# kan-bayashi/espnet

Measured on AMD Instinct MI355X. Metric: frames/sec, 12L Conformer hybrid CTC/attention training step (B=32 T=1000 d=256 per GPU), higher is better.
Workload: dtype f32; 1 GPU; BASELINE configs[1]: 12L Conformer enc d=256 h=4 ff=2048 k=31 macaron+cnn rel_pos, 6L Transformer dec, V=5000, fbank B=32 T=1000 L=100, mtlalpha 0.3, lsm 0.1; global_batch=32, frames=1000, parallelism=dp1, optimizer=adam+noam, clip 5.0, launch=hipGraph, wgrad_side_stream=False, optimizer_steps_done=114

## Files before the change

### espnet_amd/_lib.py

```python
import ctypes as C
import os

import torch

_HERE = os.path.dirname(os.path.abspath(__file__))
LIB_PATH = os.path.join(_HERE, "csrc", "libespnet_amd_hip.so")


class EamdError(RuntimeError):
    pass


class GatherT(C.Structure):
    _fields_ = [("enabled", C.c_int32), ("C", C.c_int32), ("ntap", C.c_int32), ("Ho", C.c_int32),
                ("Wo", C.c_int32), ("Hin", C.c_int32), ("Win", C.c_int32), ("sh", C.c_int32),
                ("sw", C.c_int32), ("dh", C.c_int32 * 9), ("dw", C.c_int32 * 9)]


class RowMapT(C.Structure):
    _fields_ = [("enabled", C.c_int32), ("Ho", C.c_int32), ("Wo", C.c_int32), ("Hc", C.c_int32),
                ("Wc", C.c_int32), ("sh", C.c_int32), ("oh", C.c_int32), ("sw", C.c_int32),
                ("ow", C.c_int32)]


# ... 49 lines not shown
                ("lnb_x", C.c_void_p), ("lnb_gamma", C.c_void_p), ("lnb_mean", C.c_void_p), ("lnb_rstd", C.c_void_p),
                ("lnb_dres", C.c_void_p), ("lnb_ws", C.c_void_p), ("lnb_drop_out", C.c_void_p), ("lnb_drop_salt", C.c_uint64)]


class FfnPackT(C.Structure):
    _fields_ = [("w1", C.c_void_p), ("w2", C.c_void_p), ("fwd_first", C.c_void_p), ("fwd_second", C.c_void_p),
                ("bwd_first", C.c_void_p), ("bwd_second", C.c_void_p), ("D", C.c_int32), ("F", C.c_int32)]


class RowProjPackT(C.Structure):
    _fields_ = [("w", C.c_void_p), ("image", C.c_void_p), ("K", C.c_int32), ("N", C.c_int32), ("ldw", C.c_int32),
                ("trans", C.c_int32)]


class LstmSeqFwdT(C.Structure):
    _fields_ = [("gx", C.c_void_p), ("w_hh", C.c_void_p), ("b_hh", C.c_void_p), ("live", C.c_void_p),
                ("h_out", C.c_void_p), ("c_out", C.c_void_p), ("y", C.c_void_p), ("acts", C.c_void_p),
                ("reverse", C.c_int32), ("reserved", C.c_int32)]


class LstmSeqBwdT(C.Structure):
    _fields_ = [("dy", C.c_void_p), ("w_t", C.c_void_p), ("acts", C.c_void_p), ("c_out", C.c_void_p),
                ("live", C.c_void_p), ("dgates", C.c_void_p), ("reverse", C.c_int32), ("reserved", C.c_int32)]


_lib = None

SYMBOLS = [
    "eamd_abi_version", "eamd_gemm", "eamd_gemm_multi", "eamd_gemm_group_plan", "eamd_gemm_group_launch", "eamd_ffn_fwd", "eamd_ffn_bwd", "eamd_ffn_pack_f32", "eamd_ffn_pack_bf16", "eamd_ffn_pack_f32_multi", "eamd_rowproj", "eamd_rowproj_pack_f32", "eamd_rowproj_lnb_workspace", "eamd_layernorm_fwd", "eamd_layernorm_bwd_workspace", "eamd_layernorm_bwd_drop_f32", "eamd_layernorm_bwd", "eamd_layernorm_bwd_reduce", "eamd_attn_fwd", "eamd_attn_bwd_q", "eamd_attn_fwd_f32", "eamd_attn_bwd_q_f32", "eamd_attn_bwd_kv_f32", "eamd_attn_bwd_kv", "eamd_softmax_fwd",
    "eamd_softmax_bwd", "eamd_lsm_loss", "eamd_argmax_rows", "eamd_reduce_sum", "eamd_log_softmax_rows", "eamd_transducer_expand_rows", "eamd_topk_rows", "eamd_topk_rows_i32", "eamd_weighted_topk_rows", "eamd_beam_step", "eamd_beam_step_dyn", "eamd_decode_self_attn_dyn", "eamd_beam_slots_dyn", "eamd_ctc_prefix_psi_dyn", "eamd_ctc_prefix_state_dyn", "eamd_embed_pe_dyn", "eamd_copy_jobs", "eamd_embed_pe_ld", "eamd_linear_rows_f32", "eamd_linear_rows_ln_f32", "eamd_decode_self_attn", "eamd_beam_slots", "eamd_decode_src_attn", "eamd_decode_src_attn_group", "eamd_decode_src_attn_split", "eamd_decode_src_attn_split_workspace", "eamd_weighted_sum", "eamd_beam_select", "eamd_beam_finish",
    "eamd_axpby", "eamd_cast_bf16", "eamd_scale_dev", "eamd_act_fwd", "eamd_act_bwd", "eamd_glu_fwd", "eamd_glu_bwd",
    "eamd_add_bias2", "eamd_add_cast_bf16", "eamd_add_block_f32", "eamd_add_cast_colsum2", "eamd_add_colsum2_f32", "eamd_colsum", "eamd_embed_pe", "eamd_embed_bwd", "eamd_posenc", "eamd_posenc_scaled", "eamd_posenc_scaled_bwd", "eamd_permute4",
    "eamd_dropout", "eamd_rng_advance", "eamd_dwconv_fwd", "eamd_dwconv_glu_fwd", "eamd_dwconv_glu_bwd_x", "eamd_dwconv_glu_bwd_w", "eamd_dwconv_bwd_x", "eamd_dwconv_bwd_w", "eamd_bn_nslab",
    "eamd_bn_stats", "eamd_bn_finalize", "eamd_bn_apply", "eamd_bn_bwd", "eamd_bn_stats_bounded", "eamd_bn_bwd_bounded", "eamd_mask_time", "eamd_conv1_fwd", "eamd_conv1_bwd_w_workspace", "eamd_conv1_bwd_w",
    "eamd_conv2_weight_prep", "eamd_conv2_weight_grad", "eamd_add_sos_eos", "eamd_ctc_collapse",
    "eamd_ctc_workspace_bytes", "eamd_ctc_loss", "eamd_ctc_pit_workspace_bytes", "eamd_ctc_pit_loss", "eamd_ctc_align_workspace_bytes", "eamd_ctc_forced_align", "eamd_maskctc_seed", "eamd_maskctc_update", "eamd_ctc_prefix_score", "eamd_ctc_prefix_score_batch", "eamd_ctc_prefix_psi", "eamd_ctc_prefix_state", "eamd_grad_norm", "eamd_sched_step", "eamd_adam_step", "eamd_adadelta_step", "eamd_add_gradient_noise",
    "eamd_specaug", "eamd_global_mvn", "eamd_utterance_mvn", "eamd_reflect_pad", "eamd_logmel", "eamd_unfold1d", "eamd_fold1d", "eamd_attloc_convmax_fwd", "eamd_attloc_convmax_bwd", "eamd_layernorm_bwd_drop",
    "eamd_lstm_cell_fwd", "eamd_lstm_cell_bwd", "eamd_lstm_step_fwd", "eamd_lstm_step_bwd", "eamd_lstm_seq_sync_bytes", "eamd_lstm_seq_fwd", "eamd_lstm_seq_bwd", "eamd_lstm_seq_status", "eamd_lstm_seq_status_merge", "eamd_gru_cell_fwd", "eamd_gru_cell_bwd", "eamd_maxpool2x2_fwd", "eamd_maxpool2x2_bwd", "eamd_mask_rows",
    "eamd_joint_fwd", "eamd_joint_bwd", "eamd_rnnt_workspace", "eamd_rnnt_loss", "eamd_rnnt_grad", "eamd_rnnt_node_stats", "eamd_rnnt_node_stats_part", "eamd_rnnt_row_coef", "eamd_rnnt_alpha_beta", "eamd_rnnt_node_grad",
    "eamd_conv3x3_c1_fwd", "eamd_conv3x3_c1_bwd_w_workspace", "eamd_conv3x3_c1_bwd_w", "eamd_attloc_fwd", "eamd_attloc_bwd_energy", "eamd_attloc_bwd_workspace", "eamd_attloc_bwd_energy_conv", "eamd_attloc_bwd_conv",
    "eamd_att_dot_energy_fwd", "eamd_att_dot_energy_bwd", "eamd_att_ctx_fwd", "eamd_att_ctx_bwd",
]


def lib():
    global _lib
    if _lib is None:
        if not os.path.exists(LIB_PATH):
            raise EamdError(
                f"{LIB_PATH} not found: build it with `python -c 'import __graft_entry__ as g; g.build()'` "
                "or `make -C espnet_amd/csrc` (there is no CPU fallback)")
        _lib = C.CDLL(LIB_PATH)
        _lib.eamd_ctc_workspace_bytes.restype = C.c_int64
        _lib.eamd_ctc_align_workspace_bytes.restype = C.c_int64
        _lib.eamd_ctc_pit_workspace_bytes.restype = C.c_int64
        _lib.eamd_layernorm_bwd_workspace.restype = C.c_int64
        _lib.eamd_rnnt_workspace.restype = C.c_int64
        _lib.eamd_attloc_bwd_workspace.restype = C.c_int64
        _lib.eamd_conv1_bwd_w_workspace.restype = C.c_int64
        _lib.eamd_lstm_seq_sync_bytes.restype = C.c_int64
        _lib.eamd_conv3x3_c1_bwd_w_workspace.restype = C.c_int64
        for s in SYMBOLS:
            getattr(_lib, s)
    return _lib


_raw_stream = getattr(torch._C, "_cuda_getCurrentRawStream", None)
_cur_device = getattr(torch._C, "_cuda_getDevice", None)


def stream_ptr():
    if _raw_stream is not None and _cur_device is not None:
        return C.c_void_p(_raw_stream(_cur_device()))
    return C.c_void_p(torch.cuda.current_stream().cuda_stream)


EAMD_EUNSUPPORTED = -2


def check(rc, what):
    if rc != 0:
        raise EamdError(f"{what} failed with code {rc}")


def ptr(t, offset=0):
    if t is None:
        return None
    if not t.is_cuda:
        raise EamdError("espnet_amd kernels need GPU tensors (no CPU fallback in the product path)")
    if offset == 0:
        return C.c_void_p(t.data_ptr())
    return C.c_void_p(t.data_ptr() + offset * t.element_size())


# ... 5 lines not shown
```

### espnet_amd/csrc/convmod.hip

```cpp
#include <stdlib.h>
#include "common.h"
#include "../../include/espnet_amd.h"

namespace {

constexpr int KMAX = 32;

__device__ __forceinline__ void chan_merge(float& n, float& mean, float& m2, float nb, float mb, float m2b);

template <int NWV, int MODE>
__global__ __launch_bounds__(NWV * 64) void dwconv_lds_kernel(const float* __restrict__ x, const float* __restrict__ w,
                                                              const float* __restrict__ bias, float* __restrict__ y,
                                                              int B, int T, int C, int K, int pad, int flip,
                                                              const float* __restrict__ aglu, int y_bf16,
                                                              float* __restrict__ bn_part) {
  constexpr int TB = NWV * 8;
  constexpr int NR = (TB + KMAX - 1 + NWV - 1) / NWV;
  constexpr int NWL = (64 * KMAX + NWV * 64 - 1) / (NWV * 64);
  __shared__ float xs[(TB + KMAX - 1) * 64];
  __shared__ float wl[64 * KMAX];
  const int lane = threadIdx.x & 63, wave = threadIdx.x >> 6;
  const int c0 = blockIdx.x * 64;
  const int c = min(c0 + lane, C - 1);
  const int nblk = (T + TB - 1) / TB;
// ... 402 lines not shown
  }
  sh[0][t] = s1; sh[1][t] = s2;
  __syncthreads();
  if (gi == 0 && c < C) {
    for (int g2 = 1; g2 < BN_G; ++g2) { s1 += sh[0][g2 * BN_CPB + cl]; s2 += sh[1][g2 * BN_CPB + cl]; }
    sums[c] = s1; sums[C + c] = s2;
    dbeta[c] += s1; dgamma[c] += s2;
  }
}
__global__ void bn_bwd_apply_kernel(const float* __restrict__ dy, const float* __restrict__ x,
                                    const float* __restrict__ mean, const float* __restrict__ rstd,
                                    const float* __restrict__ gamma, const float* __restrict__ beta,
                                    const float* __restrict__ sums, float* __restrict__ dx, long M, int C, int act,
                                    int training, int T, const int* __restrict__ bound) {
  const long n = M * C;
  const long stride = (long)gridDim.x * blockDim.x;
  const int tb = bound ? bound[0] : T;
  const float invM = bound ? 1.f / ((float)(M / T) * (float)tb) : 1.f / (float)M;
  for (long i = (long)blockIdx.x * blockDim.x + threadIdx.x; i < n; i += stride) {
    int c = i % C;
    if (bound && (int)((i / C) % T) >= tb) { dx[i] = 0.f; continue; }
    float rs = rstd[c], g = gamma[c];
    float xh = (x[i] - mean[c]) * rs;
    float z = xh * g + beta[c];
    float d = dy[i];
    if (act == EAMD_ACT_SWISH) d *= eamd_dswish(z);
    else if (act == EAMD_ACT_RELU) d = z > 0.f ? d : 0.f;
    else if (act != EAMD_ACT_NONE) d *= eamd_dact(z, act);
    if (training) dx[i] = g * rs * (d - sums[c] * invM - xh * sums[C + c] * invM);
    else dx[i] = g * rs * d;
  }
}

constexpr int C1_MAXF = 512;
template <int ST, int NC>
__global__ __launch_bounds__(256) void conv1_fwd_kernel(const float* __restrict__ x, const float* __restrict__ w,
                                                        const float* __restrict__ bias, float* __restrict__ y, int B,
                                                        int T, int F, int H, int W, int C, int bf16, int pad) {
  constexpr int XLD = C1_MAXF + 32;
  constexpr int NV = (ST * 7 + 3 + 3) / 4;
  __shared__ __attribute__((aligned(16))) float xs[3 * XLD];
  const int row = blockIdx.x;
  const int b = row / H, hh = row % H;
  const int FP = F + 2 * pad;
  for (int i = threadIdx.x; i < 3 * XLD; i += blockDim.x) {
    const int kh = i / XLD, j = i % XLD, f = j - pad;
    const int tt = ST * hh - pad + kh;
    const bool ok = j < FP && tt >= 0 && tt < T && f >= 0 && f < F;
    const float v = x[((long)b * T + min(max(tt, 0), T - 1)) * F + min(max(f, 0), F - 1)];
    xs[i] = ok ? v : 0.f;
  }
  __syncthreads();
  unsigned short* y16 = reinterpret_cast<unsigned short*>(y);
  unsigned int* y32 = reinterpret_cast<unsigned int*>(y);
  for (int c = threadIdx.x * NC; c < C; c += blockDim.x * NC) {
    float wr[NC][9], bv[NC];
#pragma unroll
    for (int e = 0; e < NC; ++e) {
#pragma unroll
      for (int k = 0; k < 9; ++k) wr[e][k] = w[(long)(c + e) * 9 + k];
      bv[e] = bias[c + e];
    }
    const long o = (long)row * W * C + c;
    for (int w0 = 0; w0 < W; w0 += 8) {
      float xr[3][NV * 4];
#pragma unroll
// ... 286 lines not shown
                       const float* beta, float* workspace, float* dx, float* dgamma, float* dbeta, int64_t M, int C,
                       int act, int training, int T, const int32_t* bound, void* stream) {
  if (!dy || !x || !mean || !rstd || !gamma || !beta || !workspace || !dx || !dgamma || !dbeta || M <= 0 || C <= 0)
    return EAMD_EINVAL;
  if (bound && (T <= 0 || M % T != 0)) return EAMD_EINVAL;
  if (!bn_shape_ok(C)) return EAMD_EUNSUPPORTED;
  if (((uintptr_t)x | (uintptr_t)dy | (uintptr_t)mean | (uintptr_t)rstd | (uintptr_t)gamma | (uintptr_t)beta) & 15)
    return EAMD_EINVAL;
  hipStream_t s = (hipStream_t)stream;
  const int nslab = eamd_bn_nslab(M, C);
  float* sums = workspace + (long)nslab * 2 * C;
  hipLaunchKernelGGL(bn_bwd_partial_kernel, dim3(nslab), dim3(256), 0, s, dy, x, mean, rstd, gamma, beta,
                     workspace, (long)M, C, act, T, (const int*)bound);
  EAMD_LAUNCH_CHECK();
  hipLaunchKernelGGL(bn_bwd_finalize_kernel, dim3((C + BN_CPB - 1) / BN_CPB), dim3(1024), 0, s, workspace, nslab, C, sums, dgamma, dbeta);
  EAMD_LAUNCH_CHECK();
  hipLaunchKernelGGL(bn_bwd_apply_kernel, dim3(grid_for(M * C)), dim3(256), 0, s, dy, x, mean, rstd, gamma, beta,
                     sums, dx, (long)M, C, act, training, T, (const int*)bound);
  EAMD_LAUNCH_CHECK();
  return EAMD_OK;
}
int eamd_bn_bwd(const float* dy, const float* x, const float* mean, const float* rstd, const float* gamma,
                const float* beta, float* workspace, float* dx, float* dgamma, float* dbeta, int64_t M, int C,
                int act, int training, void* stream) {
  return bn_bwd_impl(dy, x, mean, rstd, gamma, beta, workspace, dx, dgamma, dbeta, M, C, act, training, 1, nullptr, stream);
}
int eamd_bn_bwd_bounded(const float* dy, const float* x, const float* mean, const float* rstd, const float* gamma,
                        const float* beta, float* workspace, float* dx, float* dgamma, float* dbeta, int64_t M, int C,
                        int act, int training, int T, const int32_t* bound, void* stream) {
  if (!bound) return EAMD_EINVAL;
  return bn_bwd_impl(dy, x, mean, rstd, gamma, beta, workspace, dx, dgamma, dbeta, M, C, act, training, T, bound, stream);
}

static int conv_c1_fwd(const float* x, const float* w, const float* bias, void* y, int B, int T, int F, int C,
                       int y_bf16, int st, int pad, void* stream) {
  if (!x || !w || !bias || !y || B <= 0 || T + 2 * pad < 3 || F + 2 * pad < 3 || C <= 0) return EAMD_EINVAL;
  if (F + 2 * pad > C1_MAXF) return EAMD_EUNSUPPORTED;
  int H = (T + 2 * pad - 3) / st + 1, W = (F + 2 * pad - 3) / st + 1;
  hipStream_t s = (hipStream_t)stream;
  const bool pair = y_bf16 && (C % 2 == 0) && (((uintptr_t)y & 3) == 0);
  const int nthr = pair ? ((C / 2 + 63) / 64) * 64 : 256;
#define EAMD_C1F(ST_, NC_) hipLaunchKernelGGL((conv1_fwd_kernel<ST_, NC_>), dim3(B * H), dim3(min(nthr, 256)), 0, s, x, w, \
                                              bias, (float*)y, B, T, F, H, W, C, y_bf16, pad)
  if (st == 2) { if (pair) EAMD_C1F(2, 2); else EAMD_C1F(2, 1); }
  else         { if (pair) EAMD_C1F(1, 2); else EAMD_C1F(1, 1); }
#undef EAMD_C1F
  EAMD_LAUNCH_CHECK();
  return EAMD_OK;
}
int eamd_conv1_fwd(const float* x, const float* w, const float* bias, void* y, int B, int T, int F, int C,
                   int y_bf16, void* stream) {
  return conv_c1_fwd(x, w, bias, y, B, T, F, C, y_bf16, 2, 0, stream);
}
int eamd_conv3x3_c1_fwd(const float* x, const float* w, const float* bias, void* y, int B, int T, int F, int C,
                        int y_bf16, void* stream) {
  return conv_c1_fwd(x, w, bias, y, B, T, F, C, y_bf16, 1, 1, stream);
}

static void conv_c1_bwd_w_grid(int B, int H, int C, int* gx, int* gy, long* rpb) {
  long nrow = (long)B * H;
  *gx = (C + 255) / 256;
  constexpr int C1W_BLOCKS = 2048;
  long want = C1W_BLOCKS / *gx; if (want < 1) want = 1;
  *rpb = (nrow + want - 1) / want; if (*rpb < 1) *rpb = 1;
  *gy = (int)((nrow + *rpb - 1) / *rpb);
}
// ... 44 lines not shown
```

### espnet_amd/functional.py

```python
import math

import torch

from . import ops
from .ops import (ACT_NONE, ACT_RELU, ACT_SWISH, EPI_DACT_FACTOR, EPI_MUL_AUX, EPI_MUL_DSWISH, EPI_MUL_RELU_MASK, EPI_NONE,
                  EPI_RELU)


class GradSink:

    on_done = None
    on_use = None

    @staticmethod
    def use(params):
        if GradSink.on_use is not None and torch.is_grad_enabled():
            GradSink.on_use(params)
        return params

    def __init__(self, params):
        self.params = list(params)
        self.ret = [None] * len(self.params)

    def buf(self, i):
# ... 875 lines not shown
            ops.mask_time(a, T, tb)
        gl = d = bmean = None
        nbt = getattr(running_mean, "_eamd_nbt", None)
        if FUSE_GLU_DWCONV:
            d = ops.dwconv_glu_fwd(a, wd.view(Cc, K), bd_, B, T, Cc, K,
                                   bn=(bn_eps, bn_momentum, running_mean, running_var, nbt) if (training and bound is None) else None)
            if d is not None and training and bound is None:
                d, bmean, brstd = d
        if d is None:
            gl = ops.glu_fwd(a, Cc)
            d = ops.dwconv_fwd(gl, wd.view(Cc, K), bd_, B, T, Cc, K)
        if training:
            if bmean is None:
                bmean, brstd = ops.bn_stats(d, M, Cc, bn_eps, bn_momentum, running_mean, running_var, nbt, bound=bound)
        else:
            bmean = running_mean
            brstd = ops.axpby(running_var, None, 1.0, 0.0)
            brstd = torch.rsqrt_(brstd.add_(bn_eps))
        e = ops.bn_apply(d, bmean, brstd, g, be, M, Cc, act, adt)
        ctx.rp = rp
        if rp is not None:
            out = ops.rowproj(e, rp[2], Cc, bias=b2, R=x2, drop=(p_out, s_out) if p_out > 0.0 else None)
        elif p_out > 0.0 and (ops.fast() or ops.f32_epilogue_drop()):
            out = ops.linear_fwd(e, ops.wshadow(w2).view(Cc, Cc), b2, R=x2, drop=(p_out, s_out))
        elif p_out > 0.0:
            br = ops.linear_fwd(e, ops.wshadow(w2).view(Cc, Cc), b2)
            out = ops.axpby(x2, ops.dropout(br, p_out, s_out), 1.0, 1.0)
        else:
            out = ops.linear_fwd(e, ops.wshadow(w2).view(Cc, Cc), b2, R=x2 if eps is not None else None)
        ctx.save_for_backward(x2, mean, rstd, xn, a, gl, d, bmean, brstd, e)
        ctx.pr = GradSink.use(params)
        ctx.cfg = (B, T, D, Cc, K, act, training, drop)
        ctx.bound = bound
        ctx.prev = _prev_drop(x)
        return _tag_out(out.view(B, T, D), p_out, s_out)

    @staticmethod
    def backward(ctx, dout):
        x2, mean, rstd, xn, a, gl, d, bmean, brstd, e = ctx.saved_tensors
        ln_w, ln_b, w1, b1, wd, bd_, g, be, w2, b2 = ctx.pr
        B, T, D, Cc, K, act, training, (p_out, s_out) = ctx.cfg
        M = B * T
        adt = ops.act_dtype()
        sink = GradSink(ctx.pr)
        do = dout.reshape(M, D).contiguous()
        dob, g_drop = _grad_operand(dout, do, p_out, s_out)
        rp = ctx.rp if g_drop is None else None
        ops.linear_bwd_w(dob, e, sink.buf(8).view(Cc, Cc), db=sink.buf(9), a_drop=g_drop)
        if rp is not None:
            de = ops.rowproj(dob, rp[3], Cc)
        else:
            de = ops.linear_bwd_x(dob, ops.wshadow(w2).view(Cc, Cc), a_drop=g_drop)
        dd = ops.bn_bwd(de, d, bmean, brstd, g, be, sink.buf(6), sink.buf(7), M, Cc, act, training, bound=ctx.bound)
        if gl is None:
            da = ops.dwconv_glu_bwd_x(dd, wd.view(Cc, K), a, B, T, Cc, K, adt)
            if ctx.bound is not None:
                ops.mask_time(da, T, ctx.bound[1])
            ops.dwconv_glu_bwd_w(dd, a, sink.buf(4).view(Cc, K), sink.buf(5), B, T, Cc, K)
        else:
            dgl = ops.dwconv_bwd_x(dd, wd.view(Cc, K), B, T, Cc, K)
            ops.dwconv_bwd_w(dd, gl, sink.buf(4).view(Cc, K), sink.buf(5), B, T, Cc, K)
            da = ops.glu_bwd(dgl, a, Cc, adt)
            if ctx.bound is not None:
                ops.mask_time(da, T, ctx.bound[1])
        ops.linear_bwd_w(da, xn, sink.buf(2).view(2 * Cc, D), db=sink.buf(3))
        if rp is not None and da.dtype == torch.float32:
            dx = _rp_ln_bwd(da, rp[1], x2, ln_w, mean, rstd, do, sink.buf(0), sink.buf(1), ctx.prev, (B, T, D))
        else:
            dxn = ops.linear_bwd_x(da, ops.wshadow(w1).view(2 * Cc, D))
            dx = _ln_bwd_out(dxn, x2, ln_w, mean, rstd, do, sink.buf(0), sink.buf(1), ctx.prev, (B, T, D))
        return (dx, None, None, None, None, None, None, None, None) + sink.results()


_TAPS_FWD = [(kh, kw) for kh in range(3) for kw in range(3)]
_CLASSES = [((0, 0), [(0, 0), (0, 2), (2, 0), (2, 2)]), ((0, 1), [(0, 1), (2, 1)]),
            ((1, 0), [(1, 0), (1, 2)]), ((1, 1), [(1, 1)])]


def _conv3s2_fwd(y_in, w, b, B, Hi, Wi, Cc, adt):
    Ho, Wo = (Hi - 3) // 2 + 1, (Wi - 3) // 2 + 1
    wf, wd = ops.conv2_weight_prep(w, adt)
    g = ops.make_gather(Cc, _TAPS_FWD, Ho, Wo, Hi, Wi, 2, 2)
    M = B * Ho * Wo
    y = torch.empty(M, Cc, device=y_in.device, dtype=adt)
    ops.gemm(y_in, wf, y, M, Cc, 9 * Cc, 9 * Cc, Cc, Cc, transB=1, bias=b, epilogue=EPI_RELU, gather=g)
    return y, wd, Ho, Wo


def _conv3s2_bwd(dy, y_in, wd, dw_buf, db_buf, B, Hi, Wi, Ho, Wo, Cc, adt):
    dev = dy.device
    M = B * Ho * Wo
    ops.colsum(dy, db_buf)
    dwf = torch.zeros(9 * Cc, Cc, device=dev, dtype=torch.float32)
    g = ops.make_gather(Cc, _TAPS_FWD, Ho, Wo, Hi, Wi, 2, 2)
    f32_big = (not ops.fast()) and Cc % 128 == 0
    tile = 128 if f32_big else 64
    ntile = (9 * Cc // tile) * ((Cc + tile - 1) // tile)
# ... 296 lines not shown
```

### espnet_amd/ops.py

```python
import ctypes as C
import os
import math

import torch

from . import _lib
from ._lib import GatherT, GemmT, RowMapT, check, ptr, stream_ptr

ACT_NONE, ACT_RELU, ACT_SWISH = 0, 1, 2
EPI_NONE, EPI_RELU, EPI_SWISH, EPI_MUL_RELU_MASK, EPI_MUL_DSWISH, EPI_MUL_AUX, EPI_DACT_FACTOR, EPI_ROW_STATS, EPI_ROW_GRAD = 0, 1, 2, 3, 4, 5, 6, 7, 8

_PRECISIONS = {"fp32": 0, "bf16": 1}
_state = {"precision": 0}


def set_precision(name):
    if name not in _PRECISIONS:
        raise ValueError(f"precision must be one of {list(_PRECISIONS)}")
    _state["precision"] = _PRECISIONS[name]


def get_precision():
    return [k for k, v in _PRECISIONS.items() if v == _state["precision"]][0]

# ... 1470 lines not shown
    if bound is not None:
        check(_lib.lib().eamd_bn_stats_bounded(ptr(x), ptr(ws), ptr(mean), ptr(rstd), ptr(running_mean), ptr(running_var),
                                               ptr(num_batches_tracked), C.c_int64(M), Cc, C.c_float(eps), C.c_float(momentum),
                                               int(bound[0]), ptr(bound[1]), stream_ptr()), "eamd_bn_stats_bounded")
        return mean, rstd
    check(_lib.lib().eamd_bn_stats(ptr(x), ptr(ws), ptr(mean), ptr(rstd), ptr(running_mean), ptr(running_var),
                                   ptr(num_batches_tracked), C.c_int64(M), Cc, C.c_float(eps), C.c_float(momentum), stream_ptr()),
          "eamd_bn_stats")
    return mean, rstd


def bn_apply(x, mean, rstd, gamma, beta, M, Cc, act, out_dtype=torch.float32):
    y = torch.empty(x.shape, device=x.device, dtype=out_dtype)
    check(_lib.lib().eamd_bn_apply(ptr(x), ptr(mean), ptr(rstd), ptr(gamma), ptr(beta), ptr(y), C.c_int64(M), Cc,
                                   act, 1 if out_dtype == torch.bfloat16 else 0, stream_ptr()), "eamd_bn_apply")
    return y


def bn_bwd(dy, x, mean, rstd, gamma, beta, dgamma, dbeta, M, Cc, act, training, bound=None):
    nslab = _lib.lib().eamd_bn_nslab(C.c_int64(M), Cc)
    ws = torch.empty((2 * nslab + 2) * Cc, device=x.device, dtype=torch.float32)
    dx = torch.empty_like(x)
    if bound is not None:
        check(_lib.lib().eamd_bn_bwd_bounded(ptr(dy), ptr(x), ptr(mean), ptr(rstd), ptr(gamma), ptr(beta), ptr(ws), ptr(dx),
                                             ptr(dgamma), ptr(dbeta), C.c_int64(M), Cc, act, int(training), int(bound[0]),
                                             ptr(bound[1]), stream_ptr()), "eamd_bn_bwd_bounded")
        return dx
    check(_lib.lib().eamd_bn_bwd(ptr(dy), ptr(x), ptr(mean), ptr(rstd), ptr(gamma), ptr(beta), ptr(ws), ptr(dx),
                                 ptr(dgamma), ptr(dbeta), C.c_int64(M), Cc, act, int(training), stream_ptr()),
          "eamd_bn_bwd")
    return dx


def conv1_fwd(x, w, bias, B, T, F, Cc, out_dtype=torch.float32):
    H, W = (T - 3) // 2 + 1, (F - 3) // 2 + 1
    assert x.numel() == B * T * F and w.numel() == Cc * 9
    y = torch.empty(B, H, W, Cc, device=x.device, dtype=out_dtype)
    check(_lib.lib().eamd_conv1_fwd(ptr(x), ptr(w), ptr(bias), ptr(y), B, T, F, Cc,
                                    1 if out_dtype == torch.bfloat16 else 0, stream_ptr()), "eamd_conv1_fwd")
    return y


def conv1_bwd_w(dy, x, dw, db, B, T, F, Cc):
    L = _lib.lib()
    ws = torch.empty(int(L.eamd_conv1_bwd_w_workspace(B, T, Cc)), device=x.device, dtype=torch.float32)
    check(L.eamd_conv1_bwd_w(ptr(dy), ptr(x), ptr(dw), ptr(db), ptr(ws), B, T, F, Cc,
                             1 if dy.dtype == torch.bfloat16 else 0, stream_ptr()), "eamd_conv1_bwd_w")


def conv2_weight_prep(w, out_dtype=torch.float32):
    Co, Ci = w.shape[0], w.shape[1]
    wf = torch.empty(9, Ci, Co, device=w.device, dtype=out_dtype)
    wd = torch.empty(9, Co, Ci, device=w.device, dtype=out_dtype)
    check(_lib.lib().eamd_conv2_weight_prep(ptr(w), ptr(wf), ptr(wd), Co, Ci,
                                            1 if out_dtype == torch.bfloat16 else 0, stream_ptr()),
          "eamd_conv2_weight_prep")
    return wf, wd


def conv2_weight_grad(dwf, dw, Co, Ci):
    check(_lib.lib().eamd_conv2_weight_grad(ptr(dwf), ptr(dw), Co, Ci, stream_ptr()), "eamd_conv2_weight_grad")


def permute4(src, dst, dims, dst_strides, accumulate=False):
    d0, d1, d2, d3 = dims
    s0, s1, s2, s3 = dst_strides
# ... 762 lines not shown
```

### include/espnet_amd.h

```cpp
#ifndef ESPNET_AMD_H_
#define ESPNET_AMD_H_
#include <stdint.h>
#ifdef __cplusplus
extern "C" {
#endif

int eamd_abi_version(void);

typedef struct {
  int32_t enabled;
  int32_t C;
  int32_t ntap;
  int32_t Ho, Wo;
  int32_t Hin, Win;
  int32_t sh, sw;
  int32_t dh[9], dw[9];
} eamd_gather_t;

typedef struct {
  int32_t enabled;
  int32_t Ho, Wo;
  int32_t Hc, Wc;
  int32_t sh, oh, sw, ow;
} eamd_rowmap_t;
// ... 227 lines not shown
int eamd_permute4(const float* src, float* dst, int d0, int d1, int d2, int d3, int64_t s0, int64_t s1,
                  int64_t s2, int64_t s3, int accumulate, void* stream);
int eamd_dropout(const void* x, void* y, int64_t n, float p, const uint64_t* step_dev, uint64_t salt, int act,
                 int in_bf16, int out_bf16, void* stream);
int eamd_rng_advance(uint64_t* step_dev, void* stream);

int eamd_dwconv_fwd(const float* x, const float* w, const float* bias, float* y, int B, int T, int C, int K,
                    void* stream);
int eamd_dwconv_bwd_x(const float* dy, const float* w, float* dx, int B, int T, int C, int K, void* stream);
int eamd_dwconv_bwd_w(const float* dy, const float* x, float* dw, float* db, int B, int T, int C, int K,
                      void* stream);
int eamd_dwconv_glu_fwd(const float* a, const float* w, const float* bias, float* y, float* bn_part, int B, int T, int C, int K,
                        void* stream);
int eamd_dwconv_glu_bwd_x(const float* dy, const float* w, const float* a, void* da, int da_bf16, int B, int T, int C, int K,
                          void* stream);
int eamd_dwconv_glu_bwd_w(const float* dy, const float* a, float* dw, float* db, int B, int T, int C, int K, void* stream);
int eamd_bn_nslab(int64_t M, int C);
int eamd_bn_stats(const float* x, float* workspace, float* mean, float* rstd, float* running_mean,
                  float* running_var, int64_t* num_batches_tracked, int64_t M, int C, float eps, float momentum, void* stream);
int eamd_bn_finalize(const float* part, int nslab, float* mean, float* rstd, float* running_mean, float* running_var,
                     int64_t* num_batches_tracked, int C, float eps, float momentum, void* stream);
int eamd_bn_apply(const float* x, const float* mean, const float* rstd, const float* gamma, const float* beta,
                  void* y, int64_t M, int C, int act, int y_bf16, void* stream);
int eamd_bn_stats_bounded(const float* x, float* workspace, float* mean, float* rstd, float* running_mean,
                          float* running_var, int64_t* num_batches_tracked, int64_t M, int C, float eps, float momentum, int T,
                          const int32_t* bound, void* stream);
int eamd_bn_bwd_bounded(const float* dy, const float* x, const float* mean, const float* rstd, const float* gamma,
                        const float* beta, float* workspace, float* dx, float* dgamma, float* dbeta, int64_t M, int C,
                        int act, int training, int T, const int32_t* bound, void* stream);
int eamd_mask_time(void* x, int64_t rows, int C, int T, const int32_t* bound, int is_bf16, void* stream);
int eamd_bn_bwd(const float* dy, const float* x, const float* mean, const float* rstd, const float* gamma,
                const float* beta, float* workspace, float* dx, float* dgamma, float* dbeta, int64_t M, int C,
                int act, int training, void* stream);
int eamd_conv1_fwd(const float* x, const float* w, const float* bias, void* y, int B, int T, int F, int C,
                   int y_bf16, void* stream);
int64_t eamd_conv1_bwd_w_workspace(int B, int T, int C);
int eamd_conv1_bwd_w(const void* dy, const float* x, float* dw, float* db, float* workspace, int B, int T, int F,
                     int C, int dy_bf16, void* stream);

int64_t eamd_ctc_workspace_bytes(int B, int T, int Lmax);
int eamd_ctc_loss(const float* acts, int64_t stride_t, int64_t stride_b, const int64_t* ys_pad,
                  const int32_t* ilens, float* nll, float* grad, int64_t gstride_t, int64_t gstride_b,
                  void* workspace, int B, int T, int V, int Lmax, int blank, int ignore_id, float grad_scale,
                  void* stream);

int64_t eamd_ctc_pit_workspace_bytes(int S, int B, int T, int Lmax);
int eamd_ctc_pit_loss(const float* acts, const int64_t* ys_pad, const int32_t* ilens, float* nll_pair, int64_t* perm, float* pit,
                      float* grad, void* workspace, int S, int B, int T, int V, int Lmax, int blank, int ignore_id, float grad_scale,
                      void* stream);

int64_t eamd_ctc_align_workspace_bytes(int B, int T, int Lmax);
int eamd_ctc_forced_align(const float* acts, int64_t stride_t, int64_t stride_b, const int64_t* ys_pad, const int32_t* ilens,
                          float* score, int32_t* states, int64_t* tokens, int32_t* seg_start, int32_t* seg_end, void* workspace,
                          int B, int T, int V, int Lmax, int blank, int ignore_id, int normalized, void* stream);

int eamd_ctc_prefix_score(const float* logp, const float* r_prev, const int32_t* cand, const int32_t* last,
                          const int32_t* olen, float* psi, float* r_new, int nhyp, int ncand, int T, int V,
                          int blank, int eos, void* stream);

int eamd_ctc_prefix_score_batch(const float* logp, const int32_t* lens, int nutt, int per_utt, const float* r_prev,
                                const int32_t* cand, const int32_t* last, const int32_t* olen, float* psi, float* r_new,
                                int ncand, int Tmax, int V, int blank, int eos, void* stream);
int eamd_ctc_prefix_psi(const float* logp, const int32_t* lens, int nutt, int per_utt, const float* r_prev, const int32_t* cand,
                        const int32_t* last, int olen, float* psi, int ncand, int Tmax, int V, int blank, int eos, void* stream);
int eamd_ctc_prefix_state(const float* logp, const int32_t* lens, int nutt, int per_utt, const float* r_prev, const int64_t* parent,
                          const int64_t* tok, const int32_t* last, int olen, const float* alive, float* r_out, int Tmax, int V, int blank,
// ... 145 lines not shown
```

Baseline: 1.124 million frames/s.

## Fuse batchnorm backward apply into depthwise-conv GLU backward kernel

Replaces the separate BN backward, dwconv-GLU input-grad and weight-grad kernels with two kernels. The first computes the per-channel BN backward sums in one pass, using a last-arriver ticket to fold the partial slabs. The second recomputes the BN input gradient on the fly inside the depthwise conv backward and produces both the GLU input gradient and the weight and bias gradients. This avoids materializing the intermediate dd tensor and cuts kernel launches. In exchange it relies on atomic ticket synchronization, uses a shared ticket buffer across layers, and is limited to the f32, unbounded, training path.

Result: no change. 1.130 million frames/s, median of 6 (+0.5%).

```diff
diff --git a/espnet_amd/_lib.py b/espnet_amd/_lib.py
--- a/espnet_amd/_lib.py
+++ b/espnet_amd/_lib.py
@@ -105,7 +105,7 @@
     "eamd_axpby", "eamd_cast_bf16", "eamd_scale_dev", "eamd_act_fwd", "eamd_act_bwd", "eamd_glu_fwd", "eamd_glu_bwd",
     "eamd_add_bias2", "eamd_add_cast_bf16", "eamd_add_block_f32", "eamd_add_cast_colsum2", "eamd_add_colsum2_f32", "eamd_colsum", "eamd_embed_pe", "eamd_embed_bwd", "eamd_posenc", "eamd_posenc_scaled", "eamd_posenc_scaled_bwd", "eamd_permute4",
     "eamd_dropout", "eamd_rng_advance", "eamd_dwconv_fwd", "eamd_dwconv_glu_fwd", "eamd_dwconv_glu_bwd_x", "eamd_dwconv_glu_bwd_w", "eamd_dwconv_bwd_x", "eamd_dwconv_bwd_w", "eamd_bn_nslab",
-    "eamd_bn_stats", "eamd_bn_finalize", "eamd_bn_apply", "eamd_bn_bwd", "eamd_bn_stats_bounded", "eamd_bn_bwd_bounded", "eamd_mask_time", "eamd_conv1_fwd", "eamd_conv1_bwd_w_workspace", "eamd_conv1_bwd_w",
+    "eamd_bn_stats", "eamd_bn_finalize", "eamd_bn_apply", "eamd_bn_bwd", "eamd_bn_stats_bounded", "eamd_bn_bwd_bounded", "eamd_bn_bwd_sums_workspace", "eamd_bn_bwd_sums", "eamd_dwconv_glu_bn_bwd", "eamd_mask_time", "eamd_conv1_fwd", "eamd_conv1_bwd_w_workspace", "eamd_conv1_bwd_w",
     "eamd_conv2_weight_prep", "eamd_conv2_weight_grad", "eamd_add_sos_eos", "eamd_ctc_collapse",
     "eamd_ctc_workspace_bytes", "eamd_ctc_loss", "eamd_ctc_pit_workspace_bytes", "eamd_ctc_pit_loss", "eamd_ctc_align_workspace_bytes", "eamd_ctc_forced_align", "eamd_maskctc_seed", "eamd_maskctc_update", "eamd_ctc_prefix_score", "eamd_ctc_prefix_score_batch", "eamd_ctc_prefix_psi", "eamd_ctc_prefix_state", "eamd_grad_norm", "eamd_sched_step", "eamd_adam_step", "eamd_adadelta_step", "eamd_add_gradient_noise",
     "eamd_specaug", "eamd_global_mvn", "eamd_utterance_mvn", "eamd_reflect_pad", "eamd_logmel", "eamd_unfold1d", "eamd_fold1d", "eamd_attloc_convmax_fwd", "eamd_attloc_convmax_bwd", "eamd_layernorm_bwd_drop",
@@ -133,6 +133,7 @@
         _lib.eamd_conv1_bwd_w_workspace.restype = C.c_int64
         _lib.eamd_lstm_seq_sync_bytes.restype = C.c_int64
         _lib.eamd_conv3x3_c1_bwd_w_workspace.restype = C.c_int64
+        _lib.eamd_bn_bwd_sums_workspace.restype = C.c_int64
         for s in SYMBOLS:
             getattr(_lib, s)
     return _lib
diff --git a/espnet_amd/csrc/convmod.hip b/espnet_amd/csrc/convmod.hip
--- a/espnet_amd/csrc/convmod.hip
+++ b/espnet_amd/csrc/convmod.hip
@@ -458,6 +458,234 @@
   }
 }
 
+__device__ __forceinline__ float bn_dz(float d, float z, int act) {
+  if (act == EAMD_ACT_SWISH) return d * eamd_dswish(z);
+  if (act == EAMD_ACT_RELU) return z > 0.f ? d : 0.f;
+  if (act != EAMD_ACT_NONE) return d * eamd_dact(z, act);
+  return d;
+}
+constexpr int CB_NWV = 8, CB_TB = CB_NWV * 8;
+
+constexpr int FOLD_U = 16;
+__device__ __forceinline__ void slab_store(float* p, float v) {
+  __hip_atomic_store(p, v, __ATOMIC_RELAXED, __HIP_MEMORY_SCOPE_AGENT);
+}
+__device__ __forceinline__ bool last_arriver(int* ticket, int n, int* flag) {
+  asm volatile("s_waitcnt vmcnt(0)" ::: "memory");
+  __syncthreads();
+  if (threadIdx.x == 0) {
+    const int last = __hip_atomic_fetch_add(ticket, 1, __ATOMIC_RELAXED, __HIP_MEMORY_SCOPE_AGENT) == n - 1;
+    if (last) {
+      __hip_atomic_store(ticket, 0, __ATOMIC_RELAXED, __HIP_MEMORY_SCOPE_AGENT);
+      __builtin_amdgcn_fence(__ATOMIC_ACQUIRE, "agent");
+      asm volatile("s_waitcnt vmcnt(0)" ::: "memory");
+    }
+    *flag = last;
+  }
+  __syncthreads();
+  return *flag != 0;
+}
+
+__global__ __launch_bounds__(CB_NWV * 64) void bn_bwd_sums_kernel(const float* __restrict__ dy, const float* __restrict__ x,
+                                                                  const float* __restrict__ mean,
+                                                                  const float* __restrict__ rstd,
+                                                                  const float* __restrict__ gamma,
+                                                                  const float* __restrict__ beta, float* __restrict__ part,
+                                                                  int* __restrict__ ticket, float* __restrict__ sums,
+                                                                  float* __restrict__ dgamma, float* __restrict__ dbeta,
+                                                                  long M, int C, int act) {
+  constexpr int NWV = CB_NWV;
+  __shared__ float red[2][NWV][64];
+  __shared__ int is_last;
+  const int lane = threadIdx.x & 63, wave = threadIdx.x >> 6;
+  const int c0 = blockIdx.x * 64;
+  const bool clive = c0 + lane < C;
+  const int c = clive ? c0 + lane : C - 1;
+  const float mu = mean[c], rs = rstd[c], gm = gamma[c], be = beta[c];
+  const long r0 = (long)blockIdx.y * CB_TB + wave * 8;
+  float xv[8], dv[8];
+#pragma unroll
+  for (int i = 0; i < 8; ++i) {
+    const long r = min(r0 + i, M - 1);
+    xv[i] = x[r * C + c]; dv[i] = dy[r * C + c];
+  }
+  float s1 = 0.f, s2 = 0.f;
+#pragma unroll
+  for (int i = 0; i < 8; ++i) {
+    if (r0 + i < M) {
+      const float xh = (xv[i] - mu) * rs;
+      const float d = bn_dz(dv[i], xh * gm + be, act);
+      s1 += d; s2 += d * xh;
+    }
+  }
+  red[0][wave][lane] = s1; red[1][wave][lane] = s2;
+  __syncthreads();
+  if (wave == 0 && clive) {
+    for (int w2 = 1; w2 < NWV; ++w2) { s1 += red[0][w2][lane]; s2 += red[1][w2][lane]; }
+    float* pp = part + (long)blockIdx.y * 2 * C + c;
+    slab_store(pp, s1); slab_store(pp + C, s2);
+  }
+  if (!last_arriver(ticket + blockIdx.x, gridDim.y, &is_last)) return;
+  const int ny = gridDim.y;
+  const float* pc = part + c;
+  s1 = 0.f; s2 = 0.f;
+  for (int s0 = wave * FOLD_U; s0 < ny; s0 += NWV * FOLD_U) {
+    float a1[FOLD_U], a2[FOLD_U];
+#pragma unroll
+    for (int u = 0; u < FOLD_U; ++u) {
+      const long o = (long)min(s0 + u, ny - 1) * 2 * C;
+      a1[u] = pc[o]; a2[u] = pc[o + C];
+    }
+#pragma unroll
+    for (int u = 0; u < FOLD_U; ++u)
+      if (s0 + u < ny) { s1 += a1[u]; s2 += a2[u]; }
+  }
+  red[0][wave][lane] = s1; red[1][wave][lane] = s2;
+  __syncthreads();
+  if (wave == 0 && clive) {
+    for (int w2 = 1; w2 < NWV; ++w2) { s1 += red[0][w2][lane]; s2 += red[1][w2][lane]; }
+    sums[c] = s1; sums[C + c] = s2;
+    dbeta[c] += s1; dgamma[c] += s2;
+  }
+}
+
+struct BnBwdArgs {
+  const float* x;
+  const float* mean;
+  const float* rstd;
+  const float* gamma;
+  const float* beta;
+  const float* sums;
+  float inv_m;
+  int act;
+};
+__global__ __launch_bounds__(CB_NWV * 64) void dwconv_glu_bn_bwd_kernel(const float* __restrict__ dy, BnBwdArgs bn,
+                                                                        const float* __restrict__ w,
+                                                                        const float* __restrict__ a, float* __restrict__ da,
+                                                                        float* __restrict__ dw, float* __restrict__ db,
+                                                                        int B, int T, int C, int K, int pad) {
+  constexpr int NWV = CB_NWV, TB = CB_TB;
+  constexpr int HR = TB + KMAX - 1;
+  constexpr int NR = (HR + NWV - 1) / NWV;
+  constexpr int NWL = (64 * KMAX + NWV * 64 - 1) / (NWV * 64);
+  __shared__ float smem[NWV * 64 * (KMAX + 1)];
+  static_assert(2 * HR * 64 + 64 * KMAX <= NWV * 64 * (KMAX + 1), "tiles must fit in the reduction buffer");
+  float* ds = smem;
+  float* gs = smem + HR * 64;
+  float* wl = smem + 2 * HR * 64;
+  __shared__ float redb[NWV * 64];
+  const int lane = threadIdx.x & 63, wave = threadIdx.x >> 6;
+  const int c0 = blockIdx.x * 64;
+  const bool live = c0 + lane < C;
+  const int c = live ? c0 + lane : C - 1;
+  const int nblk = (T + TB - 1) / TB;
+  const int b = blockIdx.y / nblk;
+  const int tb0 = (blockIdx.y % nblk) * TB;
+  const int rows = TB + K - 1;
+  const int nw = min(64, C - c0) * K;
+  const float mu = bn.mean[c], rs = bn.rstd[c], gm = bn.gamma[c], be = bn.beta[c];
+  const float k1 = bn.sums[c] * bn.inv_m, k2 = bn.sums[C + c] * bn.inv_m, grs = gm * rs;
+  const float* eb = dy + (long)b * T * C + c;
+  const float* xb = bn.x + (long)b * T * C + c;
+  const float* ab = a + (long)b * T * 2 * C + c;
+  {
+    float ev[NR], xv[NR], vv[NR], gv[NR], tw[NWL];
+#pragma unroll
+    for (int i = 0; i < NR; ++i) {
+      const long ts = min(max(tb0 - pad + wave + i * NWV, 0), T - 1);
+      ev[i] = eb[ts * C]; xv[i] = xb[ts * C];
+      vv[i] = ab[ts * 2 * C]; gv[i] = ab[ts * 2 * C + C];
+    }
+#pragma unroll
+    for (int q = 0; q < NWL; ++q) tw[q] = w[(long)c0 * K + min((int)threadIdx.x + q * NWV * 64, nw - 1)];
+#pragma unroll
+    for (int i = 0; i < NR; ++i) {
+      const int r = wave + i * NWV, ts = tb0 - pad + r;
+      if (r < rows) {
+        const bool ok = ts >= 0 && ts < T;
+        const float xh = (xv[i] - mu) * rs;
+        const float dd = grs * (bn_dz(ev[i], xh * gm + be, bn.act) - k1 - xh * k2);
+        ds[r * 64 + lane] = ok ? dd : 0.f;
+        gs[r * 64 + lane] = ok ? vv[i] * eamd_sigmoid(gv[i]) : 0.f;
+      }
+    }
+#pragma unroll
+    for (int q = 0; q < NWL; ++q)
+      if ((int)threadIdx.x + q * NWV * 64 < nw) wl[threadIdx.x + q * NWV * 64] = tw[q];
+  }
+  __syncthreads();
+  const int t0 = tb0 + wave * 8;
+  {
+    float wr[KMAX];
+#pragma unroll
+    for (int k = 0; k < KMAX; ++k) wr[k] = (k < K) ? wl[lane * K + min(max(K - 1 - k, 0), K - 1)] : 0.f;
+    float acc[8];
+#pragma unroll
+    for (int i = 0; i < 8; ++i) acc[i] = 0.f;
+#pragma unroll
+    for (int j = 0; j < 8 + KMAX - 1; ++j) {
+      const float v = (j < 8 + K - 1) ? ds[(wave * 8 + min(j, 8 + K - 2)) * 64 + lane] : 0.f;
+#pragma unroll
+      for (int i = 0; i < 8; ++i) {
+        const int k = j - i;
+        if (k >= 0 && k < KMAX) acc[i] += wr[k] * v;
+      }
+    }
+    float av[8], gv[8];
+#pragma unroll
+    for (int i = 0; i < 8; ++i) {
+      const long r = (long)min(t0 + i, T - 1) * 2 * C;
+      av[i] = ab[r]; gv[i] = ab[r + C];
+    }
+    float* yb = da + (long)b * T * 2 * C + c;
+#pragma unroll
+    for (int i = 0; i < 8; ++i) {
+      if (!live || t0 + i >= T) continue;
+      const float sg = eamd_sigmoid(gv[i]);
+      const long r = (long)(t0 + i) * 2 * C;
+      yb[r] = acc[i] * sg;
+      yb[r + C] = acc[i] * av[i] * sg * (1.f - sg);
+    }
+  }
+  float acc[KMAX];
+#pragma unroll
+  for (int k = 0; k < KMAX; ++k) acc[k] = 0.f;
+  float accb = 0.f;
+  float g[8];
+#pragma unroll
+  for (int i = 0; i < 8; ++i) { g[i] = ds[(wave * 8 + i + pad) * 64 + lane]; accb += g[i]; }
+#pragma unroll
+  for (int j = 0; j < 8 + KMAX - 1; ++j) {
+    const float xv = (j < 8 + K - 1) ? gs[(wave * 8 + min(j, 8 + K - 2)) * 64 + lane] : 0.f;
+#pragma unroll
+    for (int i = 0; i < 8; ++i) {
+      const int k = j - i;
+      if (k >= 0 && k < KMAX) acc[k] += g[i] * xv;
+    }
+  }
+  __syncthreads();
+  float* slot = smem + wave * 64 * (KMAX + 1);
+#pragma unroll
+  for (int k = 0; k < KMAX; ++k)
+    if (k < K) slot[lane * (KMAX + 1) + k] = live ? acc[k] : 0.f;
+  redb[wave * 64 + lane] = live ? accb : 0.f;
+  __syncthreads();
+  const int nch = min(64, C - c0);
+  for (int i = threadIdx.x; i < nch * K; i += blockDim.x) {
+    const int cc = i / K, k = i % K;
+    float t = 0.f;
+#pragma unroll
+    for (int wv = 0; wv < NWV; ++wv) t += smem[wv * 64 * (KMAX + 1) + cc * (KMAX + 1) + k];
+    atomicAdd(&dw[(long)c0 * K + i], t);
+  }
+  if (db && threadIdx.x < nch) {
+    float t = 0.f;
+#pragma unroll
+    for (int wv = 0; wv < NWV; ++wv) t += redb[wv * 64 + threadIdx.x];
+    atomicAdd(&db[c0 + threadIdx.x], t);
+  }
+}
+
 constexpr int C1_MAXF = 512;
 template <int ST, int NC>
 __global__ __launch_bounds__(256) void conv1_fwd_kernel(const float* __restrict__ x, const float* __restrict__ w,
@@ -810,6 +1038,38 @@
   return bn_bwd_impl(dy, x, mean, rstd, gamma, beta, workspace, dx, dgamma, dbeta, M, C, act, training, T, bound, stream);
 }
 
+int64_t eamd_bn_bwd_sums_workspace(int64_t M, int C) {
+  if (M <= 0 || C <= 0) return 0;
+  return 2 * (int64_t)C * ((M + CB_TB - 1) / CB_TB);
+}
+
+int eamd_bn_bwd_sums(const float* dy, const float* x, const float* mean, const float* rstd, const float* gamma,
+                     const float* beta, float* workspace, int32_t* ticket, float* sums, float* dgamma, float* dbeta, int64_t M,
+                     int C, int act, void* stream) {
+  if (!dy || !x || !mean || !rstd || !gamma || !beta || !workspace || !ticket || !sums || !dgamma || !dbeta || M <= 0 || C <= 0)
+    return EAMD_EINVAL;
+  const int64_t ny = (M + CB_TB - 1) / CB_TB;
+  if (ny > 65535) return EAMD_EUNSUPPORTED;
+  hipLaunchKernelGGL(bn_bwd_sums_kernel, dim3((C + 63) / 64, (unsigned)ny), dim3(CB_NWV * 64), 0, (hipStream_t)stream, dy, x, mean,
+                     rstd, gamma, beta, workspace, (int*)ticket, sums, dgamma, dbeta, (long)M, C, act);
+  EAMD_LAUNCH_CHECK();
+  return EAMD_OK;
+}
+
+int eamd_dwconv_glu_bn_bwd(const float* dy, const float* x, const float* mean, const float* rstd, const float* gamma,
+                           const float* beta, const float* sums, const float* w, const float* a, float* da, float* dw, float* db,
+                           int B, int T, int C, int K, int act, void* stream) {
+  if (!dy || !x || !mean || !rstd || !gamma || !beta || !sums || !w || !a || !da || !dw || B <= 0 || T <= 0 || C <= 0 || K <= 0 ||
+      (K & 1) == 0)
+    return EAMD_EINVAL;
+  if (K > KMAX) return EAMD_EUNSUPPORTED;
+  const BnBwdArgs bn{x, mean, rstd, gamma, beta, sums, 1.f / ((float)B * (float)T), act};
+  hipLaunchKernelGGL(dwconv_glu_bn_bwd_kernel, dim3((C + 63) / 64, B * ((T + CB_TB - 1) / CB_TB)), dim3(CB_NWV * 64), 0,
+                     (hipStream_t)stream, dy, bn, w, a, da, dw, db, B, T, C, K, (K - 1) / 2);
+  EAMD_LAUNCH_CHECK();
+  return EAMD_OK;
+}
+
 static int conv_c1_fwd(const float* x, const float* w, const float* bias, void* y, int B, int T, int F, int C,
                        int y_bf16, int st, int pad, void* stream) {
   if (!x || !w || !bias || !y || B <= 0 || T + 2 * pad < 3 || F + 2 * pad < 3 || C <= 0) return EAMD_EINVAL;
diff --git a/espnet_amd/functional.py b/espnet_amd/functional.py
--- a/espnet_amd/functional.py
+++ b/espnet_amd/functional.py
@@ -931,6 +931,7 @@
         ctx.pr = GradSink.use(params)
         ctx.cfg = (B, T, D, Cc, K, act, training, drop)
         ctx.bound = bound
+        ctx.fused_bn = training and bound is None and gl is None and adt == torch.float32
         ctx.prev = _prev_drop(x)
         return _tag_out(out.view(B, T, D), p_out, s_out)
 
@@ -950,18 +951,22 @@
             de = ops.rowproj(dob, rp[3], Cc)
         else:
             de = ops.linear_bwd_x(dob, ops.wshadow(w2).view(Cc, Cc), a_drop=g_drop)
-        dd = ops.bn_bwd(de, d, bmean, brstd, g, be, sink.buf(6), sink.buf(7), M, Cc, act, training, bound=ctx.bound)
-        if gl is None:
-            da = ops.dwconv_glu_bwd_x(dd, wd.view(Cc, K), a, B, T, Cc, K, adt)
-            if ctx.bound is not None:
-                ops.mask_time(da, T, ctx.bound[1])
-            ops.dwconv_glu_bwd_w(dd, a, sink.buf(4).view(Cc, K), sink.buf(5), B, T, Cc, K)
-        else:
-            dgl = ops.dwconv_bwd_x(dd, wd.view(Cc, K), B, T, Cc, K)
-            ops.dwconv_bwd_w(dd, gl, sink.buf(4).view(Cc, K), sink.buf(5), B, T, Cc, K)
-            da = ops.glu_bwd(dgl, a, Cc, adt)
-            if ctx.bound is not None:
-                ops.mask_time(da, T, ctx.bound[1])
+        if ctx.fused_bn and de.dtype == torch.float32:
+            da = ops.dwconv_glu_bn_bwd(de, d, bmean, brstd, g, be, wd.view(Cc, K), a, sink.buf(6), sink.buf(7),
+                                       sink.buf(4).view(Cc, K), sink.buf(5), B, T, Cc, K, act)
+        else:
+            dd = ops.bn_bwd(de, d, bmean, brstd, g, be, sink.buf(6), sink.buf(7), M, Cc, act, training, bound=ctx.bound)
+            if gl is None:
+                da = ops.dwconv_glu_bwd_x(dd, wd.view(Cc, K), a, B, T, Cc, K, adt)
+                if ctx.bound is not None:
+                    ops.mask_time(da, T, ctx.bound[1])
+                ops.dwconv_glu_bwd_w(dd, a, sink.buf(4).view(Cc, K), sink.buf(5), B, T, Cc, K)
+            else:
+                dgl = ops.dwconv_bwd_x(dd, wd.view(Cc, K), B, T, Cc, K)
+                ops.dwconv_bwd_w(dd, gl, sink.buf(4).view(Cc, K), sink.buf(5), B, T, Cc, K)
+                da = ops.glu_bwd(dgl, a, Cc, adt)
+                if ctx.bound is not None:
+                    ops.mask_time(da, T, ctx.bound[1])
         ops.linear_bwd_w(da, xn, sink.buf(2).view(2 * Cc, D), db=sink.buf(3))
         if rp is not None and da.dtype == torch.float32:
             dx = _rp_ln_bwd(da, rp[1], x2, ln_w, mean, rstd, do, sink.buf(0), sink.buf(1), ctx.prev, (B, T, D))
diff --git a/espnet_amd/ops.py b/espnet_amd/ops.py
--- a/espnet_amd/ops.py
+++ b/espnet_amd/ops.py
@@ -1526,6 +1526,30 @@
     return dx
 
 
+_bn_tickets = {}
+
+
+def _bn_ticket(device):
+    t = _bn_tickets.get(device.index)
+    if t is None:
+        t = _bn_tickets[device.index] = torch.zeros(64, device=device, dtype=torch.int32)
+    return t
+
+
+def dwconv_glu_bn_bwd(de, d, mean, rstd, gamma, beta, w, a, dgamma, dbeta, dw, db, B, T, Cc, K, act):
+    M = B * T
+    assert de.dtype == torch.float32 and d.dtype == torch.float32 and a.dtype == torch.float32 and Cc <= 64 * 64
+    lib = _lib.lib()
+    ws = torch.empty(lib.eamd_bn_bwd_sums_workspace(C.c_int64(M), Cc), device=d.device, dtype=torch.float32)
+    sums = torch.empty(2 * Cc, device=d.device, dtype=torch.float32)
+    check(lib.eamd_bn_bwd_sums(ptr(de), ptr(d), ptr(mean), ptr(rstd), ptr(gamma), ptr(beta), ptr(ws), ptr(_bn_ticket(d.device)),
+                               ptr(sums), ptr(dgamma), ptr(dbeta), C.c_int64(M), Cc, act, stream_ptr()), "eamd_bn_bwd_sums")
+    da = torch.empty(M, 2 * Cc, device=d.device, dtype=torch.float32)
+    check(lib.eamd_dwconv_glu_bn_bwd(ptr(de), ptr(d), ptr(mean), ptr(rstd), ptr(gamma), ptr(beta), ptr(sums), ptr(w), ptr(a),
+                                     ptr(da), ptr(dw), ptr(db), B, T, Cc, K, act, stream_ptr()), "eamd_dwconv_glu_bn_bwd")
+    return da
+
+
 def conv1_fwd(x, w, bias, B, T, F, Cc, out_dtype=torch.float32):
     H, W = (T - 3) // 2 + 1, (F - 3) // 2 + 1
     assert x.numel() == B * T * F and w.numel() == Cc * 9
diff --git a/include/espnet_amd.h b/include/espnet_amd.h
--- a/include/espnet_amd.h
+++ b/include/espnet_amd.h
@@ -283,6 +283,13 @@
 int eamd_bn_bwd(const float* dy, const float* x, const float* mean, const float* rstd, const float* gamma,
                 const float* beta, float* workspace, float* dx, float* dgamma, float* dbeta, int64_t M, int C,
                 int act, int training, void* stream);
+int64_t eamd_bn_bwd_sums_workspace(int64_t M, int C);
+int eamd_bn_bwd_sums(const float* dy, const float* x, const float* mean, const float* rstd, const float* gamma,
+                     const float* beta, float* workspace, int32_t* ticket, float* sums, float* dgamma, float* dbeta, int64_t M,
+                     int C, int act, void* stream);
+int eamd_dwconv_glu_bn_bwd(const float* dy, const float* x, const float* mean, const float* rstd, const float* gamma,
+                           const float* beta, const float* sums, const float* w, const float* a, float* da, float* dw, float* db,
+                           int B, int T, int C, int K, int act, void* stream);
 int eamd_conv1_fwd(const float* x, const float* w, const float* bias, void* y, int B, int T, int F, int C,
                    int y_bf16, void* stream);
 int64_t eamd_conv1_bwd_w_workspace(int B, int T, int C);
```
